# kmjc/PulsePortraiture

Measured on AMD Instinct MI355X. Metric: TOAs/sec (phase+DM fit, 64ch×2048bin fp64) at 1/2/4/8 MI355X, higher is better.
Workload: dtype f64

## Files before the change

include/ppfit.h:

```cpp
#ifndef PPFIT_H
#define PPFIT_H

#include <stdint.h>

#ifdef __cplusplus
extern "C" {
#endif

#define PPF_OK 0
#define PPF_ERR_INVALID -1
#define PPF_ERR_DEVICE -2
#define PPF_ERR_UNSUPPORTED -3
#define PPF_ERR_NOMEM -4

#define PPF_MAX_NCHAN 16384
#define PPF_LDS_NCHAN 2048
#define PPF_VERSION 1

#define PPF_K_MODEL_FFT 0
#define PPF_K_DATA_XSPEC 1
#define PPF_K_SOLVE 2
#define PPF_K_PHASE_SHIFT 3
#define PPF_K_ROTATE 4
#define PPF_K_ROT_ACCUM 5
// ... 17 lines not shown
typedef struct ppf_ctx ppf_ctx;

int ppf_version(void);
int ppf_ctx_create(int device, ppf_ctx** out);
void ppf_ctx_destroy(ppf_ctx* ctx);
const char* ppf_last_error(const ppf_ctx* ctx);
int ppf_set_stream(ppf_ctx* ctx, void* stream);
int ppf_synchronize(ppf_ctx* ctx);
int ppf_set_pipeline(ppf_ctx* ctx, int32_t pieces);
#define PPF_OPT_SCAT_GRAPH 0
#define PPF_OPT_SCAT_SPLIT 1
#define PPF_OPT_SCAT_TAIL 2
#define PPF_OPT_FUSE_MOMENTS 3
#define PPF_OPT_GUESS_WAVE 4
#define PPF_OPT_HBM_TABLES 5
#define PPF_NUM_OPTS 6
int ppf_set_option(ppf_ctx* ctx, int32_t option, int32_t value);
int ppf_get_option(const ppf_ctx* ctx, int32_t option, int32_t* value);
int ppf_set_workspace_limit(ppf_ctx* ctx, int64_t bytes);
int ppf_get_workspace_limit(const ppf_ctx* ctx, int64_t* bytes);
int ppf_set_timing(ppf_ctx* ctx, int enable);
int ppf_set_trace(ppf_ctx* ctx, double* buf, int32_t cap);
int ppf_get_kernel_time(ppf_ctx* ctx, int kernel_id, double* total_ms,
                        int64_t* launches);
int ppf_reset_kernel_times(ppf_ctx* ctx);
int ppf_get_pca_gram_times(ppf_ctx* ctx, double* ms);
#define PPF_SELFTEST_N 10
int ppf_selftest(ppf_ctx* ctx, int32_t* fails);
#define PPF_PHASE_N 32
int ppf_phase_profile(ppf_ctx* ctx, int32_t enable, uint64_t* out);

// ... 247 lines not shown
```

pulseportraiture_amd/_lib.py:

```python
import ctypes
import os

HERE = os.path.dirname(os.path.abspath(__file__))
LIB_PATH = os.path.join(HERE, "libppfit.so")

PPF_OK = 0
PPF_METHOD_TRUST_NCG = 0
PPF_METHOD_TNC = 1
PPF_METHOD_NEWTON_CG = 2
PPF_METHOD_TNC_LEGACY = 3
METHODS = {"trust-ncg": PPF_METHOD_TRUST_NCG, "TNC": PPF_METHOD_TNC,
           "Newton-CG": PPF_METHOD_NEWTON_CG, "TNC-legacy": PPF_METHOD_TNC_LEGACY}
KERNEL_IDS = {"model_fft": 0, "data_xspec": 1, "solve": 2, "phase_shift": 3,
              "rotate": 4, "rot_accum": 5, "synth": 6, "irfft": 7, "noise": 8,
              "guess": 9, "post": 10, "fit_taylor": 11, "moments": 12, "resid": 13, "unpack": 14,
              "pca": 15, "gauss": 16, "pack": 17, "swt": 18, "gbank": 19, "fscrunch": 20}
PPF_THRESH = {"hard": 0, "soft": 1}
PPF_SOLVE_EXACT = 1
PPF_SOLVE_EVAL = 2
PPF_GUESS_DIRECT = 4
PPF_SPEC_NONE = 0
PPF_SPEC_STORE = 1
PPF_SPEC_USE = 2
PPF_SELFTEST_N = 10
GAUSS_STATUS = {1: "converged: ftol", 2: "converged: xtol", 3: "converged: ftol and xtol",
                5: "evaluation cap reached", -1: "singular normal equations",
                -2: "non-finite residual"}
OPTIONS = {"scat_graph": 0, "scat_split": 1, "scat_tail": 2, "fuse_moments": 3, "guess_wave": 4,
           "hbm_tables": 5}
PPF_PHASE_N = 32

_dp = ctypes.c_void_p


class FitDesc(ctypes.Structure):
    _fields_ = [("nsub", ctypes.c_int32), ("nchan", ctypes.c_int32),
                ("nbin", ctypes.c_int32), ("nmodel", ctypes.c_int32),
                ("fit_flags", ctypes.c_int32 * 5),
                ("log10_tau", ctypes.c_int32), ("option", ctypes.c_int32),
                ("method", ctypes.c_int32), ("is_toa", ctypes.c_int32),
                ("guess", ctypes.c_int32), ("guess_Ns", ctypes.c_int32),
                ("guess_wrap", ctypes.c_int32), ("solver_flags", ctypes.c_int32),
                ("data", _dp), ("model", _dp), ("model_idx", _dp),
                ("freqs", _dp), ("errs", _dp), ("chan_mask", _dp),
# ... 149 lines not shown
```

pulseportraiture_amd/build.py:

```python
import hashlib
import os
import subprocess
import sys

HERE = os.path.dirname(os.path.abspath(__file__))
ROOT = os.path.dirname(HERE)
CSRC = os.path.join(HERE, "csrc")
INC = os.path.join(ROOT, "include")
HIPCC = os.environ.get("HIPCC", "/opt/rocm/bin/hipcc")
CXX = os.environ.get("CXX", "g++")

SOURCES = ["ppfit_lib.hip"]
DEPS = ["ppfit_lib.hip", "ppfit_spectra.hip", "ppfit_fit.hip", "ppfit_taylor.hip", "ppfit_tnc.hip",
        "ppfit_ncg.hip", "ppfit_models.hip", "ppfit_generic.hip", "ppfit_noisefit.hip", "ppfit_fscrunch.hip", "ppfit_fake.hip", "ppfit_pca.hip",
        "ppfit_gram.hip",
        "ppfit_gauss.hip", "ppfit_gbank.hip", "ppfit_swt.hip", "ppfit_nbscat.hip", "ppfit_capi.hip",
        "ppfit_kernels.hpp", "ppfit_device.hpp"]
OUT = os.path.join(HERE, "libppfit.so")
FITS_OUT = os.path.join(HERE, "libppfits.so")
TIM_OUT = os.path.join(HERE, "libpptim.so")

HASH_TAG = b"PPF_SRC_HASH="


def _lib_specs():
    hip = ([HIPCC, "--offload-arch=gfx950", "-O3", "-std=c++17", "-fPIC", "-shared", "-I" + INC,
            "-I" + CSRC, os.path.join(CSRC, SOURCES[0])],
           [os.path.join(CSRC, f) for f in DEPS] + [os.path.join(INC, "ppfit.h")])
    fits = ([CXX, "-O2", "-std=c++17", "-fPIC", "-shared", "-Wall", "-I" + INC,
             os.path.join(CSRC, "psrfits.cpp"), os.path.join(CSRC, "psrfits_write.cpp")],
            [os.path.join(CSRC, "psrfits.cpp"), os.path.join(CSRC, "psrfits_write.cpp"),
             os.path.join(INC, "ppfits.h"), os.path.join(INC, "ppfitsw.h")])
# ... 63 lines not shown
```

pulseportraiture_amd/csrc/ppfit_capi.hip:

```cpp
#include <hip/hip_runtime.h>

#include <algorithm>
#include <cmath>
#include <cstdarg>
#include <cstdio>
#include <cstdlib>
#include <cstring>
#include <string>
#include <vector>

#include "ppfit.h"
#include "ppfit_kernels.hpp"

#ifndef PPF_SRC_HASH
#define PPF_SRC_HASH "unbuilt"
#endif
extern "C" __attribute__((visibility("default"), used)) const char ppf_build_tag[] =
    "PPF_SRC_HASH=" PPF_SRC_HASH;

using namespace ppf;

namespace {

struct TimedLaunch {
// ... 30 lines not shown
  int64_t ws_limit = (int64_t)32 << 30;
  TableCache tw, vp;
  Buffer buf[kNumBuffers];
  size_t taylor_static_lds = kUnknown;
  int* active_h = nullptr;
  hipEvent_t scat_ev[2] = {nullptr, nullptr};
  hipStream_t stream2 = nullptr;
  int pipe = 0;
  std::vector<hipEvent_t> sync_events;
  bool phase_prof = false;
  bool timing = false;
  std::vector<TimedLaunch> pending;
  std::vector<hipEvent_t> pool;
  double* trace = nullptr;
  int trace_cap = 0;
  int opt[PPF_NUM_OPTS] = {1, 1, 512, 1, 1, 0};
  double ktime[PPF_NUM_KERNELS] = {0};
  int64_t klaunch[PPF_NUM_KERNELS] = {0};
  double gram_ms[5] = {0.0, 0.0, 0.0, 0.0, 0.0};
};

namespace {

int fail(ppf_ctx* ctx, int code, const char* fmt, ...) {
  char buf[512];
  va_list ap;
  va_start(ap, fmt);
  vsnprintf(buf, sizeof(buf), fmt, ap);
  va_end(ap);
  if (ctx) ctx->err = buf;
  return code;
// ... 341 lines not shown
  return timed_on(ctx, PPF_K_FIT_TAYLOR, st, [&] {
    WIDE_SWITCH(L.wide, {
      if (fa.Dsp) {
        if (mom) hipLaunchKernelGGL((k_fit_taylor<true, true, WD>), g, b, lds, st, fa);
        else hipLaunchKernelGGL((k_fit_taylor<false, true, WD>), g, b, lds, st, fa);
      } else {
        if (mom) hipLaunchKernelGGL((k_fit_taylor<true, false, WD>), g, b, lds, st, fa);
        else hipLaunchKernelGGL((k_fit_taylor<false, false, WD>), g, b, lds, st, fa);
      }
    });
  });
}

int stage_post(ppf_ctx* ctx, hipStream_t st, int n, const FitArgs& fa, const FitLaunch& L) {
  return timed_on(ctx, PPF_K_POST, st, [&] {
    WIDE_SWITCH(L.wide, {
      hipLaunchKernelGGL((k_post<false, WD>), dim3(n), dim3(kBlock), L.lds_meta, st, fa);
      hipLaunchKernelGGL((k_post<true, WD>), dim3(n), dim3(kBlock), L.lds_meta, st, fa);
    });
  });
}

int stage_errs(ppf_ctx* ctx, hipStream_t st, int n, const SpecArgs& sa, double* errs_out) {
  if (!errs_out) return PPF_OK;
  HIPCHK(ctx, hipMemcpyAsync(errs_out + (size_t)sa.sub0 * sa.nchan, sa.sig,
                             (size_t)n * sa.nchan * sizeof(double), hipMemcpyDeviceToDevice, st));
  return PPF_OK;
}

int scat_split_solve(ppf_ctx* ctx, const FitArgs& fa, int nc, int split, size_t lds_scat) {
  const int nchan = fa.nchan;
  double* part = static_cast<double*>(ctx->buf[kSpart].p);
// ... 355 lines not shown
  const bool exact = fit_is_exact(d), taylor = fit_is_taylor(d);
  SpecArgs sa{};
  FitArgs fa{};
  bind_fit_args(ctx, d, o, sa, fa);
  if (int r = fit_tables(ctx, d, sa, fa)) return r;

  const bool wide = nchan > PPF_LDS_NCHAN || ctx->opt[PPF_OPT_HBM_TABLES] != 0;
  FitWorkspace ws(nchan, fa.NHP, taylor, wide, ctx->ws_limit, d->nsub);
  if (int r = ensure(ctx, ctx->buf[kWs], ws.total)) return r;
  ws.base = static_cast<char*>(ctx->buf[kWs].p);
  ws.slice(0, sa, fa);
  const int64_t chunk = ws.chunk;

  L.nbin = nbin;
  L.wide = wide;
  L.lds_meta = wide ? 0 : meta_lds(nchan);
  L.lds_xspec = wide ? 0 : xspec_dyn_lds(nchan);
  fa.tnl = taylor && !wide ? taylor_lds_moments(ctx, nchan, L.lds_meta) : 0;
  fa.tlds = fa.tnl > 0 ? (int)L.lds_meta : 0;
  L.lds_taylor = L.lds_meta + (size_t)nchan * fa.tnl * sizeof(double);
  L.lds_guess =
      (size_t)(fa.NHP + (d->guess ? pfa_scratch_slots(d->guess_Ns, NH) : 0)) * sizeof(double2);
  const bool split_scat = ctx->opt[PPF_OPT_SCAT_SPLIT] && d->fit_flags[3] &&
                          d->method == PPF_METHOD_TRUST_NCG && !wide;
  const int split = std::max(1, std::min(16, nchan / 64));
  L.lds_scat = scat_sweep_lds(nchan, split);
  if (split_scat) {
    if (int r = ensure(ctx, ctx->buf[kSpart],
                       (size_t)chunk * ((nchan + 7) / 8) * kScatPart * sizeof(double) +
                           64 * sizeof(int) + 256))
// ... 1669 lines not shown
```

pulseportraiture_amd/csrc/ppfit_fit.hip:

```cpp
#include "ppfit_kernels.hpp"

namespace ppf {

constexpr int NACC = 10;
static_assert(NACC == kScatAcc, "k_scat_sweep's LDS rows (scat_sweep_lds)");
constexpr double kTwoPi = 2.0 * kPi;
constexpr double kFourPi2 = 4.0 * kPi * kPi;
constexpr double kDconst2 = kDconst * kDconst;

__host__ __device__ constexpr int pair_i(int p) {
  return p < 5 ? 0 : (p < 9 ? 1 : (p < 12 ? 2 : (p < 14 ? 3 : 4)));
}
__host__ __device__ constexpr int pair_j(int p) {
  return p < 5 ? p : (p < 9 ? p - 4 : (p < 12 ? p - 7 : (p < 14 ? p - 9 : 4)));
}

struct Meta {
  int* chan;
  double* fr;
  double* iw2;
  double* pn;
  double* d1;
  double* d2;
  int nok;
};

__device__ __forceinline__ size_t meta_bytes(int nchan) {
  return (size_t)nchan * (5 * sizeof(double) + sizeof(int));
}

__device__ Meta load_meta(const FitArgs& a, int c, int s, unsigned char* dyn, int* s_nok) {
  Meta m;
  const int nchan = a.nchan;
  m.fr = reinterpret_cast<double*>(dyn);
  m.iw2 = m.fr + nchan;
  m.pn = m.iw2 + nchan;
  m.d1 = m.pn + nchan;
  m.d2 = m.d1 + nchan;
  m.chan = reinterpret_cast<int*>(m.d2 + nchan);
  const int tid = threadIdx.x, lane = tid & 63;
  const uint8_t* mask = a.mask ? a.mask + (size_t)s * nchan : nullptr;
  if (tid < 64) {
    int base = 0;
    for (int n0 = 0; n0 < nchan; n0 += 64) {
      const int n = n0 + lane;
// ... 1 lines not shown
      const unsigned long long b = __ballot(ok);
      const int rank = __popcll(b & ((1ull << lane) - 1ull));
      if (ok) m.chan[base + rank] = n;
      base += __popcll(b);
    }
    if (lane == 0) *s_nok = base;
  }
  __syncthreads();
  m.nok = *s_nok;
  const int midx = a.model_idx ? a.model_idx[s] : 0;
  const double half = 0.5 * (double)a.nbin;
  const double P = a.P[s];
  const double* refs = a.st[c].refs;
  const double r0 = 1.0 / (refs[0] * refs[0]);
  const double r1 = 1.0 / (refs[1] * refs[1]);
  for (int j = tid; j < m.nok; j += kBlock) {
    const int n = m.chan[j];
    const double fr = a.freqs[(size_t)s * nchan + n];
    m.fr[j] = fr;
    const double sg = a.sig[(size_t)c * nchan + n];
    m.iw2[j] = 1.0 / (sg * sg * half);
    m.pn[j] = a.pn[(size_t)midx * nchan + n];
    const double f2 = 1.0 / (fr * fr);
    m.d1[j] = kDconst * (f2 - r0) / P;
    m.d2[j] = kDconst2 * (f2 * f2 - r1 * r1) / P;
  }
  __syncthreads();
  return m;
}

__device__ __forceinline__ double pymod1(double x) {
// ... 16 lines not shown
__device__ __forceinline__ void block_sum_vec(double (&v)[N], double (*red)[48]) {
  const int lane = threadIdx.x & 63, w = threadIdx.x >> 6;
#pragma unroll
  for (int i = 0; i < N; ++i) {
    const double t = wave_sum(v[i]);
    if (lane == 0) red[w][i] = t;
  }
  __syncthreads();
#pragma unroll
  for (int i = 0; i < N; ++i) {
    double t = 0.0;
    for (int q = 0; q < kWaves; ++q) t += red[q][i];
    v[i] = t;
  }
  __syncthreads();
}

constexpr int kPipe = 4;

#ifndef PPF_SCAT_U
#define PPF_SCAT_U 4
#endif
#ifndef PPF_SCAT_WG_PER_CU
#define PPF_SCAT_WG_PER_CU 3
#endif

__device__ __forceinline__ void cells_phase(const double2* __restrict__ Xr, int J, int h,
                                            double phif, double* acc) {
  const double2 step = turn_phasor(8.0, phif);
  const double2 zero = cmk(0.0, 0.0);
// ... 345 lines not shown
    ym *= y8;
  }
  double r0, i1, r2;
  switch (h & 3) {
    case 1: r0 = -S0; i1 = S1; r2 = -S2; break;
    case 2: r0 = -S0; i1 = -S1; r2 = -S2; break;
    case 3: r0 = S0; i1 = -S1; r2 = S2; break;
    default: r0 = S0; i1 = S1; r2 = S2; break;
  }
  acc[0] = r0;
  acc[1] = Ks * i1;
  acc[2] = (Ks * Ks) * r2;
  for (int i = 3; i < NACC; ++i) acc[i] = 0.0;
}

__device__ double taylor_reach(const Meta& m, const double* prm, const double* refs,
                               const TaylorSrc& ts, double P, double Ks, double* red) {
  double mx = 0.0;
  for (int j = threadIdx.x; j < m.nok; j += kBlock)
    mx = fmax(mx, fabs(ts.same ? taylor_delta_lin(prm, ts.xc, m.d1[j], m.d2[j])
                               : taylor_delta(prm, refs, ts, m.fr[j], P)));
  mx = wave_max(mx);
  const int lane = threadIdx.x & 63, w = threadIdx.x >> 6;
  if (lane == 0) red[w] = mx;
  __syncthreads();
  double r = red[0];
  for (int i = 1; i < kWaves; ++i) r = fmax(r, red[i]);
  __syncthreads();
  return kTwoPi * Ks * r;
}

__device__ __forceinline__ int flag_mask(const FitArgs& a) {
  int fm = 0;
#pragma unroll
  for (int i = 0; i < 5; ++i) fm |= a.flags[i] ? 1 << i : 0;
  return fm;
}
// ... 61 lines not shown
    bool on = true;
    if (tid == 0) src = 0;
    else if (tid < 4) { src = tid; on = (fm >> (tid - 1)) & 1; }
    else if (tid >= 6) {
      const int p = tid - 6, pi = pair_i(p), pj = pair_j(p);
      if (pj < 3) { src = 4 + (pi == 0 ? pj : 1 + pi + pj); on = (fm >> pi) & (fm >> pj) & 1; }
    }
    double v = 0.0;
    if (src >= 0 && on)
      for (int q = 0; q < kWaves; ++q) v += red[q][src];
    out[tid] = v;
  }
  __syncthreads();
}

template <int MODE, bool SCAT>
__device__ __forceinline__ void sweep(const FitArgs& a, const Meta& m, int c, int s, const double* prm,
                      const double* refs, double P, double* acc_slot, double* out,
                      double (*red)[48], const TaylorSrc& ts, double (*lrow)[48] = nullptr) {
  if constexpr (MODE == 0 && !SCAT) {
    if (ts.T && ts.same) {
      sweep_taylor0(a, m, prm, acc_slot, out, red, ts);
      return;
    }
  }
  const int tid = threadIdx.x, lane = tid & 63, w = tid >> 6;
  const int g8 = lane >> 3, h = lane & 7;
  const int J = a.NHP >> 3;
  const bool log10_tau = a.log10_tau != 0;
  const double tau_lin = SCAT ? (log10_tau ? pow(10.0, prm[3]) : prm[3]) : 0.0;
  const bool scat = SCAT && tau_lin != 0.0;
  const int midx = a.model_idx ? a.model_idx[s] : 0;
  const int fm = flag_mask(a);
  constexpr int NP = MODE == 0 ? 21 : 45;
  double* myrow = nullptr;
  if (lane < NP) red[w][lane] = 0.0;
  if constexpr (MODE == 1) {
    myrow = lrow[w * 8 + g8];
    if (h == 0)
      for (int i = 0; i < NP; ++i) myrow[i] = 0.0;
  }
  __syncthreads();
  const int ngroups = (m.nok + 7) >> 3;
  for (int gi = w; gi < ngroups; gi += kWaves) {
    const int j = gi * 8 + g8;
    const bool valid = j < m.nok;
    const int jj = valid ? j : m.nok - 1;
    const int n = m.chan[jj];
    const double fr = m.fr[jj];
    double acc[NACC];
    if (!SCAT && ts.T) {
      const double dl = ts.same ? taylor_delta_lin(prm, ts.xc, m.d1[jj], m.d2[jj])
                                : taylor_delta(prm, refs, ts, fr, P);
      taylor_cells(ts, n, h, dl, 0.5 * (double)a.nbin, acc);
    } else if (!scat) {
      const double phif = phase_frac(prm, fr, refs, P);
      const double2* Xr = a.X + ((size_t)c * a.nchan + n) * a.NHP;
      cells_phase(Xr, J, h, phif, acc);
    } else {
      const double phif = phase_frac(prm, fr, refs, P);
      const double2* Xr = a.X + ((size_t)c * a.nchan + n) * a.NHP;
      const double* M2r = a.M2 + ((size_t)midx * a.nchan + n) * a.NHP;
      const double taun = tau_lin * pow(fr / refs[2], prm[4]);
      cells_scat<PPF_SCAT_U>(Xr, M2r, J, h, phif, taun, acc);
    }
#pragma unroll
    for (int i = 0; i < NACC; ++i) acc[i] = group8_sum(acc[i]);
    if constexpr (MODE == 0) {
      const double dpre[2] = {m.d1[jj], m.d2[jj]};
      const ChanDeriv d = derive<SCAT>(acc, scat, m.pn[jj], m.iw2[jj], fr, prm, tau_lin, refs,
                                       P, log10_tau, dpre);
      const double q = d.C * d.C / d.S;
      const LanePick L{d.dph[0], d.dph[1], d.dph[2], d.dts[0],
                       d.dts[1], d.d2ts[0], d.d2ts[1], d.d2ts[2]};
      if (h == 0 && valid) {
        double* dst = acc_slot + (size_t)j * NACC;
        for (int i = 0; i < NACC; ++i) dst[i] = acc[i];
      }
#pragma unroll
      for (int r = 0; r < 3; ++r) {
        const double v = chan8_sum(valid ? mode0_term(d, L, q, h + 8 * r, fm) : 0.0);
        const int t = (lane & 7) + 8 * r;
        if (lane >= 8 && lane < 16 && t < NP) red[w][t] += v;
      }
    } else {
      double ct[NP];
#pragma unroll
      for (int i = 0; i < NP; ++i) ct[i] = 0.0;
      if (h == 0 && valid) {
        const ChanDeriv d = derive<SCAT>(acc, scat, m.pn[j], m.iw2[j], fr, prm, tau_lin, refs, P,
                                         log10_tau);
        const double q = d.C * d.C / d.S;
        const double sc = d.C / d.S;
        double cross[5];
#pragma unroll
        for (int i = 0; i < 5; ++i) cross[i] = -2.0 * (dC_(d, i) - sc * dS_(d, i));
        double* dst = a.wsc + ((size_t)c * a.nchan + j) * 8;
        dst[0] = sc;
        dst[1] = d.S;
#pragma unroll
        for (int i = 0; i < 5; ++i) dst[2 + i] = cross[i];
        const double ic = 1.0 / (2.0 * d.S);
#pragma unroll
        for (int p = 0; p < 15; ++p) {
          const int pi = pair_i(p), pj = pair_j(p);
          if (a.flags[pi] && a.flags[pj]) {
            ct[p] = -2.0 * q * ((d2C_(d, pi, pj) / d.C) - (0.5 * d2S_(d, pi, pj) / d.S));
            ct[15 + p] = cross[pi] * cross[pj] * ic;
            ct[30 + p] = Hn_(d, pi, pj);
          }
        }
      }
      if (h == 0 && valid)
#pragma unroll
        for (int i = 0; i < NP; ++i) myrow[i] += ct[i];
    }
  }
  __syncthreads();
  if (tid < NP) {
    double t = 0.0;
    if constexpr (MODE == 0)
      for (int q = 0; q < kWaves; ++q) t += red[q][tid];
    else
      for (int r = 0; r < kWaves * 8; ++r) t += lrow[r][tid];
    out[tid] = t;
  }
  __syncthreads();
}

__device__ __forceinline__ bool fused_taylor(const FitArgs& a, int s) {
  if (!a.T) return false;
  const double t3 = a.init[(size_t)s * 5 + 3];
  const double tl = a.log10_tau ? pow(10.0, t3) : t3;
  return !((tl != 0.0) || a.flags[3]);
}

// ... 1077 lines not shown
    default: break;
  }
}

__device__ __forceinline__ int nz_nsums(int br) {
  switch (br) {
    case NZ_PD: case NZ_PG: case NZ_TA: return 2;
    case NZ_PDT: return 6;
    case NZ_PDG: return 8;
    case NZ_PDGT: return 14;
    case NZ_PDTA: return 22;
    default: return 0;
  }
}

template <int N>
__device__ __forceinline__ void block_sum_first(double (&v)[22], double (*red)[48]) {
  double u[N];
#pragma unroll
  for (int i = 0; i < N; ++i) u[i] = v[i];
  block_sum_vec(u, red);
#pragma unroll
  for (int i = 0; i < N; ++i) v[i] = u[i];
}

__device__ double closest_positive(const double* r, int nr, bool sq, double fmean) {
  double best = NAN, bd = INFINITY;
  for (int i = 0; i < nr; ++i) {
    if (!(r[i] > 0.0)) continue;
    const double x = sq ? sqrt(r[i]) : r[i];
    const double dd = fabs(fmean - x);
    if (dd < bd) { bd = dd; best = x; }
  }
  return best;
}

__device__ int nz_solve(int br, int option, const double* t, double* nz, PostWs& w) {
  switch (br) {
// ... 51 lines not shown
          co[2] = -(A * A * b - a * a * B) - H44 * C * d - H14 * E * f + H44 * b * E +
                  (A * C * f - a * c * F) + H14 * A * d;
          co[3] = 2 * A * a * b + H44 * c * d + H14 * e * f - H44 * b * e - (A * c + a * C) * f -
                  H14 * a * d;
          co[4] = -a * a * b + a * c * f;
          deg = 4;
        }
        return deg;
      }
    } break;
    default: break;
  }
  return 0;
}

struct PostShared {
  PostWs ws;
  double lrow[kWaves * 8][48];
  double prm[5], refs[3], nu[3];
  double out[48];
  double red[kWaves][48];
  double Xinv[25];
  double ifact[kMT];
  int ifit[5];
  int nfit, nok, bad;
  double fmean, Sd;
};

template <bool SCAT, bool W>
__device__ void post_subint(const FitArgs& a, int c, int s, unsigned char* dyn, PostShared& sh) {
  const int tid = threadIdx.x;
  const int nchan = a.nchan;
  const bool prof = a.ptime != nullptr;
  unsigned long long t0 = prof ? wall_clock64() : 0ull;
  auto mark = [&](int i) {
    if (prof) {
      const unsigned long long t1 = wall_clock64();
      if (tid == 0) atomicAdd(&a.ptime[i], t1 - t0);
      t0 = t1;
    }
  };
  const Meta m = load_meta(a, c, s, dyn, &sh.nok);
  const SolveState& st = a.st[c];
  const double P = a.P[s];
  const bool log10_tau = a.log10_tau != 0;
  if (a.mask) {
    for (int n = tid; n < nchan; n += kBlock) {
      if (a.mask[(size_t)s * nchan + n]) continue;
      const size_t o = (size_t)s * nchan + n;
      a.o_scales[o] = 0.0;
      a.o_scale_errs[o] = 0.0;
      a.o_channel_snrs[o] = 0.0;
    }
  }
  {
    double v[2] = {0.0, 0.0};
    for (int j = tid; j < m.nok; j += kBlock) {
      v[0] += a.dsum[(size_t)c * nchan + m.chan[j]] * m.iw2[j];
      v[1] += m.fr[j];
    }
    block_sum_vec(v, sh.red);
    if (tid == 0) { sh.Sd = v[0]; sh.fmean = v[1] / (double)m.nok; }
  }
  if (tid == 0) {
    sh.nfit = 0;
    for (int i = 0; i < 5; ++i) if (a.flags[i]) sh.ifit[sh.nfit++] = i;
    for (int i = 0; i < 3; ++i) sh.refs[i] = st.refs[i];
    sh.bad = (m.nok == 0);
  }
  __syncthreads();
  mark(16);
  if (sh.bad) {
    if (tid == 0) {
      for (int i = 0; i < 5; ++i) {
        a.o_params[(size_t)s * 5 + i] = NAN;
        a.o_param_errs[(size_t)s * 5 + i] = NAN;
      }
// ... 5 lines not shown
  const double* acc_fin = a.acc + ((size_t)c * 2 + st.slot) * nchan * NACC;
  bool need = false;
  double nuo[3];
  for (int i = 0; i < 3; ++i) {
    nuo[i] = a.nu_out[(size_t)s * 3 + i];
    if (isnan(nuo[i]) || nuo[i] == 0.0) need = true;
  }
  if (need) {
    int fl[5];
    for (int i = 0; i < 5; ++i) fl[i] = a.flags[i] ? 1 : 0;
    const int br = nz_branch(fl);
    if (br == NZ_PDTA) fl[2] = 0;
    double t[22];
    double sums[22];
    for (int i = 0; i < 22; ++i) sums[i] = 0.0;
    if (br != NZ_NONE) {
      const double tau_lin = log10_tau ? pow(10.0, st.x[3]) : st.x[3];
      const bool scat = SCAT && tau_lin != 0.0;
      for (int j = tid; j < m.nok; j += kBlock) {
        const ChanDeriv d = derive<SCAT>(acc_fin + (size_t)j * NACC, scat, m.pn[j], m.iw2[j], m.fr[j],
                                   st.x, tau_lin, sh.refs, P, log10_tau);
        nz_terms(br, a.option, d, m.fr[j], sh.refs, fl, t);
        for (int i = 0; i < 22; ++i) sums[i] += t[i];
      }
    }
    switch (nz_nsums(br)) {
      case 2: block_sum_first<2>(sums, sh.red); break;
      case 6: block_sum_first<6>(sums, sh.red); break;
      case 8: block_sum_first<8>(sums, sh.red); break;
      case 14: block_sum_first<14>(sums, sh.red); break;
      case 22: block_sum_first<22>(sums, sh.red); break;
      default: break;
    }
    double* nz = sh.ws.nz;
    if (tid == 0) {
      for (int i = 0; i < 3; ++i) nz[i] = sh.refs[i];
      sh.ws.deg = nz_solve(br, a.option, sums, nz, sh.ws);
    }
    __syncthreads();
    const int pdeg = sh.ws.deg;
    if (pdeg > 0) {
      const int nr = poly_real_roots(sh.ws.co, pdeg, sh.ws, tid);
      if (tid == 0) nz[0] = nz[1] = closest_positive(sh.ws.prev, nr, true, sh.fmean);
    }
    if (tid == 0)
      for (int i = 0; i < 3; ++i) if (isnan(nuo[i])) nuo[i] = nz[i];
  }
// ... 19 lines not shown
    sh.prm[2] = x[2];
    sh.prm[3] = tau_out;
    sh.prm[4] = x[4];
    for (int i = 0; i < 3; ++i) sh.nu[i] = nuo[i];
  }
  __syncthreads();
  TaylorSrc ts{};
  if (!SCAT && st.taylor) {
    const double Ks = 0.5 * (double)a.nbin;
    if (tid < kMT) sh.ifact[tid] = c_inv_fact[tid];
    int best = st.xslot;
    double by = INFINITY;
    for (int q = 0; q < 2; ++q) {
      if (!(st.mvalid & (1 << q))) continue;
      const TaylorSrc tq{a.T + ((size_t)c * 2 + q) * nchan * kMT, st.xc[q], st.refs};
      const double y = taylor_reach(m, sh.prm, sh.nu, tq, P, Ks, sh.red[0]);
      if (y < by) { by = y; best = q; }
    }
    ts = TaylorSrc{a.T + ((size_t)c * 2 + best) * nchan * kMT, st.xc[best], st.refs, false,
                   sh.ifact};
  }
  mark(18);
  sweep<1, SCAT>(a, m, c, s, sh.prm, sh.nu, P, nullptr, sh.out, sh.red, ts, sh.lrow);
  mark(19);
  if (tid == 0) {
    bool fit[5];
#pragma unroll
    for (int i = 0; i < 5; ++i) fit[i] = a.flags[i] != 0;
    double A[5][5], Ai[5][5];
#pragma unroll
    for (int p = 0; p < 15; ++p) {
      const int pi = pair_i(p), pj = pair_j(p);
      A[pi][pj] = A[pj][pi] = sh.out[p] - sh.out[15 + p];
    }
    const bool ok = invert5_fitted(A, fit, Ai);
#pragma unroll
    for (int i = 0; i < 5; ++i)
#pragma unroll
// ... 16 lines not shown
        int r = 0;
#pragma unroll
        for (int j = 0; j < 5; ++j) {
          if (!fit[j]) continue;
          cn[q * 5 + r] = okc ? Ai[i][j] : NAN;
          ++r;
        }
        ++q;
      }
    }
  }
  __syncthreads();
  mark(20);
  const int nf = sh.nfit;
  double snr2 = 0.0;
  for (int j = tid; j < m.nok; j += kBlock) {
    const double* w = a.wsc + ((size_t)c * nchan + j) * 8;
    const double sc = w[0], S = w[1];
    const double ic = 1.0 / (2.0 * S);
    double LL[5], U[5];
#pragma unroll
    for (int q = 0; q < 5; ++q) U[q] = a.flags[q] ? w[2 + q] : 0.0;
#pragma unroll
    for (int q = 0; q < 5; ++q) {
      double t = 0.0;
#pragma unroll
      for (int i = 0; i < 5; ++i)
        if (a.flags[i] && a.flags[q]) t += U[i] * sh.Xinv[i * 5 + q];
      LL[q] = -ic * t;
    }
    double t = 0.0;
#pragma unroll
    for (int q = 0; q < 5; ++q)
      if (a.flags[q]) t += LL[q] * U[q];
    const double LR = -t * ic + ic;
    const double csnr = sc * sqrt(S);
    const int n = m.chan[j];
    const size_t o = (size_t)s * nchan + n;
    a.o_scales[o] = sc;
    a.o_scale_errs[o] = sqrt(2.0 * LR);
    a.o_channel_snrs[o] = csnr;
    snr2 += csnr * csnr;
  }
  snr2 = block_sum(snr2, sh.red[0]);
  if (tid == 0) {
    double* op = a.o_params + (size_t)s * 5;
    double* oe = a.o_param_errs + (size_t)s * 5;
    for (int i = 0; i < 5; ++i) { op[i] = sh.prm[i]; oe[i] = 0.0; }
    double* cv = a.o_cov + (size_t)s * 25;
    for (int i = 0; i < 25; ++i) cv[i] = 0.0;
    int q = 0;
    for (int i = 0; i < 5; ++i) {
      if (!a.flags[i]) continue;
      oe[i] = sqrt(2.0 * sh.Xinv[i * 5 + i]);
      int r = 0;
      for (int j = 0; j < 5; ++j) {
        if (!a.flags[j]) continue;
        cv[q * 5 + r] = 2.0 * sh.Xinv[i * 5 + j];
        ++r;
// ... 9 lines not shown
    a.o_nfev[s] = st.nfev;
    a.o_status[s] = st.status;
    if (a.o_init_used) for (int i = 0; i < 5; ++i) a.o_init_used[(size_t)s * 5 + i] = st.init[i];
    if (a.o_fun) a.o_fun[s] = st.fun;
  }
  mark(21);
  if (prof && tid == 0) atomicAdd(&a.ptime[22], 1ull);
}

template <bool SCAT, bool WIDE>
#ifndef PPF_POST_SCAT_WG_PER_CU
#define PPF_POST_SCAT_WG_PER_CU 2
#endif
__global__ __launch_bounds__(kBlock, SCAT ? PPF_POST_SCAT_WG_PER_CU : PPF_POST_WG_PER_CU) void k_post(FitArgs a) {
  extern __shared__ __align__(16) unsigned char dyn[];
  __shared__ PostShared sh;
  const int c = blockIdx.x, s = a.sub0 + c;
  if ((a.st[c].scat_post != 0) != SCAT) return;
  post_subint<SCAT, WIDE>(a, c, s, chan_tables<WIDE>(a, dyn), sh);
}

}
```

pulseportraiture_amd/csrc/ppfit_kernels.hpp:

```cpp
#pragma once
#include "ppfit.h"
#include "ppfit_device.hpp"

namespace ppf {

struct SpecArgs {
  int sub0, nchan, NHP, kc, guess;
  int log10_tau, fit_tau, exact;
  int spec_mode;
  const double* data;
  const double2* M;
  const int* model_idx;
  const double* freqs;
  const double* errs;
  const uint8_t* mask;
  const double* weights;
  const double* P;
  const double* init;
  const double* guess_nu;
  double2* X;
  double2* R;
  double* sig;
  double* dsum;
  const double2* tw;
// ... 57 lines not shown
  int taylor;
  double xc[2][5];
  int mvalid, xslot;
  double g[5], H[25], tr;
  double xp[5], pl[5], predv;
  int hits, kit, sdone;
};

struct FitArgs {
  int sub0, nchan, nbin, NH, NHP, kc;
  int flags[5];
  int log10_tau, option, is_toa, guess, Ns, guess_wrap;
  int solver_flags;
  int method;
  int guess_wave;
  const double2* X;
  const double2* Dsp;
  const double2* R;
  const double2* M;
  const double* M2;
  const double* pn;
  const int* model_idx;
  const double* sig;
  const double* dsum;
  const double* freqs;
  const uint8_t* mask;
  const double* P;
  const double* init;
  const double* nu_fit;
  const double* nu_out;
// ... 20 lines not shown
  double* o_channel_snrs;
  double* o_chi2;
  double* o_red_chi2;
  double* o_snr;
  int* o_nfev;
  int* o_status;
  double* o_init_used;
  double* o_fun;
  double* o_cov_nosc;
  double* o_grad;
  double* o_hess;
  double bounds[5][2];
  unsigned char* gdyn;
  size_t gdyn_stride;
};

constexpr int kTraceRec = 32;
__device__ __forceinline__ void trace_sweep(const FitArgs& a, int s, int isweep, const double* x,
                                            const double* out, int nout, bool counted) {
  if (!a.trace || threadIdx.x != 0 || isweep >= a.trace_cap) return;
  double* r = a.trace + ((size_t)s * a.trace_cap + isweep) * kTraceRec;
  for (int i = 0; i < 5; ++i) r[i] = x[i];
  for (int i = 0; i < 21; ++i) r[5 + i] = i < nout ? out[i] : NAN;
  r[26] = counted ? 1.0 : 0.0;
  r[27] = (double)isweep;
}

struct GuessShared {
  double red[kWaves];
  double bestv[kWaves];
// ... 635 lines not shown
  return scat_meta_lds(nchan) + rows * (kScatAcc * sizeof(double) + 2 * sizeof(double));
}
__global__ void k_scat_sweep(FitArgs a, double* part, int split, int init);
__global__ void k_scat_step(FitArgs a, const double* part, int init, int* ctrs, int par);
__global__ void k_model_mean(const double2* M, double2* Mmean, int nchan, int NHP);
template <bool MOM, bool DSP, bool WIDE = false>
__global__ void k_fit_taylor(FitArgs a);
template <int U, bool DSP>
__global__ void k_moments(FitArgs a);
__global__ void k_selftest(int* fails);
template <bool SCAT, bool WIDE = false> __global__ void k_solve(FitArgs a);
template <bool SCAT, bool WIDE = false> __global__ void k_tnc(FitArgs a);
template <bool SCAT, bool WIDE = false> __global__ void k_ncg(FitArgs a);
__global__ void k_guess_w(FitArgs a);
template <bool SCAT, bool WIDE = false> __global__ void k_post(FitArgs a);

}
```

Measured before the change: 1.266 million.

## Run non-scattering post stage on single-wave workgroups via virtual-thread emulation

Adds a 64-thread k_post_w kernel that handles the non-scattering post-fit stage for small channel counts when Taylor tables are present and tau is not fitted. Each wave loops over virtual wave slots, so the block-wide reductions and syncs become wave-level sums. The point is to stop wasting a full block with heavy LDS on only 64 channels and to raise occupancy. The cost is serialised slot loops within one wave, plus a duplicate code path controlled by a new option that is on by default.

Measured after the change: 1.305 million, median of 6. 3.1% higher.

```diff
diff --git a/include/ppfit.h b/include/ppfit.h
--- a/include/ppfit.h
+++ b/include/ppfit.h
@@ -55,7 +55,8 @@
 #define PPF_OPT_FUSE_MOMENTS 3
 #define PPF_OPT_GUESS_WAVE 4
 #define PPF_OPT_HBM_TABLES 5
-#define PPF_NUM_OPTS 6
+#define PPF_OPT_POST_WAVE 6
+#define PPF_NUM_OPTS 7
 int ppf_set_option(ppf_ctx* ctx, int32_t option, int32_t value);
 int ppf_get_option(const ppf_ctx* ctx, int32_t option, int32_t* value);
 int ppf_set_workspace_limit(ppf_ctx* ctx, int64_t bytes);
diff --git a/pulseportraiture_amd/_lib.py b/pulseportraiture_amd/_lib.py
--- a/pulseportraiture_amd/_lib.py
+++ b/pulseportraiture_amd/_lib.py
@@ -27,7 +27,7 @@
                 5: "evaluation cap reached", -1: "singular normal equations",
                 -2: "non-finite residual"}
 OPTIONS = {"scat_graph": 0, "scat_split": 1, "scat_tail": 2, "fuse_moments": 3, "guess_wave": 4,
-           "hbm_tables": 5}
+           "hbm_tables": 5, "post_wave": 6}
 PPF_PHASE_N = 32
 
 _dp = ctypes.c_void_p
diff --git a/pulseportraiture_amd/build.py b/pulseportraiture_amd/build.py
--- a/pulseportraiture_amd/build.py
+++ b/pulseportraiture_amd/build.py
@@ -15,7 +15,7 @@
         "ppfit_ncg.hip", "ppfit_models.hip", "ppfit_generic.hip", "ppfit_noisefit.hip", "ppfit_fscrunch.hip", "ppfit_fake.hip", "ppfit_pca.hip",
         "ppfit_gram.hip",
         "ppfit_gauss.hip", "ppfit_gbank.hip", "ppfit_swt.hip", "ppfit_nbscat.hip", "ppfit_capi.hip",
-        "ppfit_kernels.hpp", "ppfit_device.hpp"]
+        "ppfit_kernels.hpp", "ppfit_device.hpp", "ppfit_vthread.hpp"]
 OUT = os.path.join(HERE, "libppfit.so")
 FITS_OUT = os.path.join(HERE, "libppfits.so")
 TIM_OUT = os.path.join(HERE, "libpptim.so")
diff --git a/pulseportraiture_amd/csrc/ppfit_capi.hip b/pulseportraiture_amd/csrc/ppfit_capi.hip
--- a/pulseportraiture_amd/csrc/ppfit_capi.hip
+++ b/pulseportraiture_amd/csrc/ppfit_capi.hip
@@ -68,7 +68,7 @@
   std::vector<hipEvent_t> pool;
   double* trace = nullptr;
   int trace_cap = 0;
-  int opt[PPF_NUM_OPTS] = {1, 1, 512, 1, 1, 0};
+  int opt[PPF_NUM_OPTS] = {1, 1, 512, 1, 1, 0, 1};
   double ktime[PPF_NUM_KERNELS] = {0};
   int64_t klaunch[PPF_NUM_KERNELS] = {0};
   double gram_ms[5] = {0.0, 0.0, 0.0, 0.0, 0.0};
@@ -440,8 +440,10 @@
 
 int stage_post(ppf_ctx* ctx, hipStream_t st, int n, const FitArgs& fa, const FitLaunch& L) {
   return timed_on(ctx, PPF_K_POST, st, [&] {
+    if (post_wave_ok(fa)) hipLaunchKernelGGL(k_post_w, dim3(n), dim3(64), L.lds_meta, st, fa);
     WIDE_SWITCH(L.wide, {
-      hipLaunchKernelGGL((k_post<false, WD>), dim3(n), dim3(kBlock), L.lds_meta, st, fa);
+      if (!post_wave_ok(fa))
+        hipLaunchKernelGGL((k_post<false, WD>), dim3(n), dim3(kBlock), L.lds_meta, st, fa);
       hipLaunchKernelGGL((k_post<true, WD>), dim3(n), dim3(kBlock), L.lds_meta, st, fa);
     });
   });
@@ -827,6 +829,7 @@
 
   L.nbin = nbin;
   L.wide = wide;
+  fa.post_wave = ctx->opt[PPF_OPT_POST_WAVE] && !wide;
   L.lds_meta = wide ? 0 : meta_lds(nchan);
   L.lds_xspec = wide ? 0 : xspec_dyn_lds(nchan);
   fa.tnl = taylor && !wide ? taylor_lds_moments(ctx, nchan, L.lds_meta) : 0;
diff --git a/pulseportraiture_amd/csrc/ppfit_fit.hip b/pulseportraiture_amd/csrc/ppfit_fit.hip
--- a/pulseportraiture_amd/csrc/ppfit_fit.hip
+++ b/pulseportraiture_amd/csrc/ppfit_fit.hip
@@ -1,4 +1,5 @@
 #include "ppfit_kernels.hpp"
+#include "ppfit_vthread.hpp"
 
 namespace ppf {
 
@@ -29,6 +30,7 @@
   return (size_t)nchan * (5 * sizeof(double) + sizeof(int));
 }
 
+template <int NT = kBlock>
 __device__ Meta load_meta(const FitArgs& a, int c, int s, unsigned char* dyn, int* s_nok) {
   Meta m;
   const int nchan = a.nchan;
@@ -60,7 +62,7 @@
   const double* refs = a.st[c].refs;
   const double r0 = 1.0 / (refs[0] * refs[0]);
   const double r1 = 1.0 / (refs[1] * refs[1]);
-  for (int j = tid; j < m.nok; j += kBlock) {
+  for (int j = tid; j < m.nok; j += NT) {
     const int n = m.chan[j];
     const double fr = a.freqs[(size_t)s * nchan + n];
     m.fr[j] = fr;
@@ -107,6 +109,24 @@
     v[i] = t;
   }
   __syncthreads();
+}
+
+template <int NT, int N>
+__device__ __forceinline__ void vt_sum_vec(double (&v)[N], double (&tot)[N], double (*red)[48]) {
+  if constexpr (NT == kBlock) {
+    block_sum_vec(v, red);
+#pragma unroll
+    for (int i = 0; i < N; ++i) tot[i] = v[i];
+  } else {
+#pragma unroll
+    for (int i = 0; i < N; ++i) tot[i] += wave_sum(v[i]);
+  }
+}
+
+template <int NT>
+__device__ __forceinline__ double vt_sum(double v, double tot, double* red) {
+  if constexpr (NT == kBlock) return block_sum(v, red);
+  else return tot + wave_sum(v);
 }
 
 constexpr int kPipe = 4;
@@ -482,13 +502,15 @@
   for (int i = 3; i < NACC; ++i) acc[i] = 0.0;
 }
 
+template <int NT = kBlock>
 __device__ double taylor_reach(const Meta& m, const double* prm, const double* refs,
                                const TaylorSrc& ts, double P, double Ks, double* red) {
   double mx = 0.0;
-  for (int j = threadIdx.x; j < m.nok; j += kBlock)
+  for (int j = threadIdx.x; j < m.nok; j += NT)
     mx = fmax(mx, fabs(ts.same ? taylor_delta_lin(prm, ts.xc, m.d1[j], m.d2[j])
                                : taylor_delta(prm, refs, ts, m.fr[j], P)));
   mx = wave_max(mx);
+  if constexpr (NT == 64) return kTwoPi * Ks * mx;
   const int lane = threadIdx.x & 63, w = threadIdx.x >> 6;
   if (lane == 0) red[w] = mx;
   __syncthreads();
@@ -580,17 +602,19 @@
   __syncthreads();
 }
 
-template <int MODE, bool SCAT>
+template <int MODE, bool SCAT, int NT = kBlock>
 __device__ __forceinline__ void sweep(const FitArgs& a, const Meta& m, int c, int s, const double* prm,
                       const double* refs, double P, double* acc_slot, double* out,
                       double (*red)[48], const TaylorSrc& ts, double (*lrow)[48] = nullptr) {
+  static_assert(NT == kBlock || (MODE == 1 && kBlock % NT == 0 && NT % 64 == 0),
+                "only the with-scales sweep runs on virtual waves");
   if constexpr (MODE == 0 && !SCAT) {
     if (ts.T && ts.same) {
       sweep_taylor0(a, m, prm, acc_slot, out, red, ts);
       return;
     }
   }
-  const int tid = threadIdx.x, lane = tid & 63, w = tid >> 6;
+  const int tid = threadIdx.x, lane = tid & 63, rw = tid >> 6;
   const int g8 = lane >> 3, h = lane & 7;
   const int J = a.NHP >> 3;
   const bool log10_tau = a.log10_tau != 0;
@@ -600,92 +624,105 @@
   const int fm = flag_mask(a);
   constexpr int NP = MODE == 0 ? 21 : 45;
   double* myrow = nullptr;
-  if (lane < NP) red[w][lane] = 0.0;
-  if constexpr (MODE == 1) {
-    myrow = lrow[w * 8 + g8];
-    if (h == 0)
-      for (int i = 0; i < NP; ++i) myrow[i] = 0.0;
-  }
-  __syncthreads();
   const int ngroups = (m.nok + 7) >> 3;
-  for (int gi = w; gi < ngroups; gi += kWaves) {
-    const int j = gi * 8 + g8;
-    const bool valid = j < m.nok;
-    const int jj = valid ? j : m.nok - 1;
-    const int n = m.chan[jj];
-    const double fr = m.fr[jj];
-    double acc[NACC];
-    if (!SCAT && ts.T) {
-      const double dl = ts.same ? taylor_delta_lin(prm, ts.xc, m.d1[jj], m.d2[jj])
-                                : taylor_delta(prm, refs, ts, fr, P);
-      taylor_cells(ts, n, h, dl, 0.5 * (double)a.nbin, acc);
-    } else if (!scat) {
-      const double phif = phase_frac(prm, fr, refs, P);
-      const double2* Xr = a.X + ((size_t)c * a.nchan + n) * a.NHP;
-      cells_phase(Xr, J, h, phif, acc);
-    } else {
-      const double phif = phase_frac(prm, fr, refs, P);
-      const double2* Xr = a.X + ((size_t)c * a.nchan + n) * a.NHP;
-      const double* M2r = a.M2 + ((size_t)midx * a.nchan + n) * a.NHP;
-      const double taun = tau_lin * pow(fr / refs[2], prm[4]);
-      cells_scat<PPF_SCAT_U>(Xr, M2r, J, h, phif, taun, acc);
-    }
-#pragma unroll
-    for (int i = 0; i < NACC; ++i) acc[i] = group8_sum(acc[i]);
-    if constexpr (MODE == 0) {
-      const double dpre[2] = {m.d1[jj], m.d2[jj]};
-      const ChanDeriv d = derive<SCAT>(acc, scat, m.pn[jj], m.iw2[jj], fr, prm, tau_lin, refs,
-                                       P, log10_tau, dpre);
-      const double q = d.C * d.C / d.S;
-      const LanePick L{d.dph[0], d.dph[1], d.dph[2], d.dts[0],
-                       d.dts[1], d.d2ts[0], d.d2ts[1], d.d2ts[2]};
-      if (h == 0 && valid) {
-        double* dst = acc_slot + (size_t)j * NACC;
-        for (int i = 0; i < NACC; ++i) dst[i] = acc[i];
-      }
-#pragma unroll
-      for (int r = 0; r < 3; ++r) {
-        const double v = chan8_sum(valid ? mode0_term(d, L, q, h + 8 * r, fm) : 0.0);
-        const int t = (lane & 7) + 8 * r;
-        if (lane >= 8 && lane < 16 && t < NP) red[w][t] += v;
-      }
-    } else {
-      double ct[NP];
-#pragma unroll
-      for (int i = 0; i < NP; ++i) ct[i] = 0.0;
-      if (h == 0 && valid) {
-        const ChanDeriv d = derive<SCAT>(acc, scat, m.pn[j], m.iw2[j], fr, prm, tau_lin, refs, P,
-                                         log10_tau);
+  const int nslot = NT == kBlock ? 1 : vt_live_slots(ngroups, kWaves, NT / 64);
+  double tot = 0.0;
+  for (int sl = 0; sl < nslot; ++sl) {
+    const int w = vt_wave(rw, sl, NT);
+    if constexpr (NT == kBlock)
+      if (lane < NP) red[w][lane] = 0.0;
+    if constexpr (MODE == 1) {
+      myrow = lrow[NT == kBlock ? ws_row(w, g8) : ws_local_row(rw, g8)];
+      if (h == 0)
+        for (int i = 0; i < NP; ++i) myrow[i] = 0.0;
+    }
+    __syncthreads();
+    for (int gi = ws_first_group(w); gi < ngroups; gi += kWaves) {
+      const int j = gi * 8 + g8;
+      const bool valid = j < m.nok;
+      const int jj = valid ? j : m.nok - 1;
+      const int n = m.chan[jj];
+      const double fr = m.fr[jj];
+      double acc[NACC];
+      if (!SCAT && ts.T) {
+        const double dl = ts.same ? taylor_delta_lin(prm, ts.xc, m.d1[jj], m.d2[jj])
+                                  : taylor_delta(prm, refs, ts, fr, P);
+        taylor_cells(ts, n, h, dl, 0.5 * (double)a.nbin, acc);
+      } else if (!scat) {
+        const double phif = phase_frac(prm, fr, refs, P);
+        const double2* Xr = a.X + ((size_t)c * a.nchan + n) * a.NHP;
+        cells_phase(Xr, J, h, phif, acc);
+      } else {
+        const double phif = phase_frac(prm, fr, refs, P);
+        const double2* Xr = a.X + ((size_t)c * a.nchan + n) * a.NHP;
+        const double* M2r = a.M2 + ((size_t)midx * a.nchan + n) * a.NHP;
+        const double taun = tau_lin * pow(fr / refs[2], prm[4]);
+        cells_scat<PPF_SCAT_U>(Xr, M2r, J, h, phif, taun, acc);
+      }
+#pragma unroll
+      for (int i = 0; i < NACC; ++i) acc[i] = group8_sum(acc[i]);
+      if constexpr (MODE == 0) {
+        const double dpre[2] = {m.d1[jj], m.d2[jj]};
+        const ChanDeriv d = derive<SCAT>(acc, scat, m.pn[jj], m.iw2[jj], fr, prm, tau_lin, refs,
+                                         P, log10_tau, dpre);
         const double q = d.C * d.C / d.S;
-        const double sc = d.C / d.S;
-        double cross[5];
-#pragma unroll
-        for (int i = 0; i < 5; ++i) cross[i] = -2.0 * (dC_(d, i) - sc * dS_(d, i));
-        double* dst = a.wsc + ((size_t)c * a.nchan + j) * 8;
-        dst[0] = sc;
-        dst[1] = d.S;
-#pragma unroll
-        for (int i = 0; i < 5; ++i) dst[2 + i] = cross[i];
-        const double ic = 1.0 / (2.0 * d.S);
-#pragma unroll
-        for (int p = 0; p < 15; ++p) {
-          const int pi = pair_i(p), pj = pair_j(p);
-          if (a.flags[pi] && a.flags[pj]) {
-            ct[p] = -2.0 * q * ((d2C_(d, pi, pj) / d.C) - (0.5 * d2S_(d, pi, pj) / d.S));
-            ct[15 + p] = cross[pi] * cross[pj] * ic;
-            ct[30 + p] = Hn_(d, pi, pj);
+        const LanePick L{d.dph[0], d.dph[1], d.dph[2], d.dts[0],
+                         d.dts[1], d.d2ts[0], d.d2ts[1], d.d2ts[2]};
+        if (h == 0 && valid) {
+          double* dst = acc_slot + (size_t)j * NACC;
+          for (int i = 0; i < NACC; ++i) dst[i] = acc[i];
+        }
+#pragma unroll
+        for (int r = 0; r < 3; ++r) {
+          const double v = chan8_sum(valid ? mode0_term(d, L, q, h + 8 * r, fm) : 0.0);
+          const int t = (lane & 7) + 8 * r;
+          if (lane >= 8 && lane < 16 && t < NP) red[w][t] += v;
+        }
+      } else {
+        double ct[NP];
+#pragma unroll
+        for (int i = 0; i < NP; ++i) ct[i] = 0.0;
+        if (h == 0 && valid) {
+          const ChanDeriv d = derive<SCAT>(acc, scat, m.pn[j], m.iw2[j], fr, prm, tau_lin, refs, P,
+                                           log10_tau);
+          const double q = d.C * d.C / d.S;
+          const double sc = d.C / d.S;
+          double cross[5];
+#pragma unroll
+          for (int i = 0; i < 5; ++i) cross[i] = -2.0 * (dC_(d, i) - sc * dS_(d, i));
+          double* dst = a.wsc + ((size_t)c * a.nchan + j) * 8;
+          dst[0] = sc;
+          dst[1] = d.S;
+#pragma unroll
+          for (int i = 0; i < 5; ++i) dst[2 + i] = cross[i];
+          const double ic = 1.0 / (2.0 * d.S);
+#pragma unroll
+          for (int p = 0; p < 15; ++p) {
+            const int pi = pair_i(p), pj = pair_j(p);
+            if (a.flags[pi] && a.flags[pj]) {
+              ct[p] = -2.0 * q * ((d2C_(d, pi, pj) / d.C) - (0.5 * d2S_(d, pi, pj) / d.S));
+              ct[15 + p] = cross[pi] * cross[pj] * ic;
+              ct[30 + p] = Hn_(d, pi, pj);
+            }
           }
         }
-      }
-      if (h == 0 && valid)
-#pragma unroll
-        for (int i = 0; i < NP; ++i) myrow[i] += ct[i];
-    }
-  }
-  __syncthreads();
+        if (h == 0 && valid)
+#pragma unroll
+          for (int i = 0; i < NP; ++i) myrow[i] += ct[i];
+      }
+    }
+    __syncthreads();
+    if constexpr (NT < kBlock) {
+      if (tid < NP)
+        for (int r = 0; r < (NT / 64) * 8; ++r) tot += lrow[r][tid];
+      __syncthreads();
+    }
+  }
   if (tid < NP) {
     double t = 0.0;
-    if constexpr (MODE == 0)
+    if constexpr (NT < kBlock)
+      t = tot;
+    else if constexpr (MODE == 0)
       for (int q = 0; q < kWaves; ++q) t += red[q][tid];
     else
       for (int r = 0; r < kWaves * 8; ++r) t += lrow[r][tid];
@@ -1793,14 +1830,15 @@
   }
 }
 
-template <int N>
-__device__ __forceinline__ void block_sum_first(double (&v)[22], double (*red)[48]) {
-  double u[N];
-#pragma unroll
-  for (int i = 0; i < N; ++i) u[i] = v[i];
-  block_sum_vec(u, red);
-#pragma unroll
-  for (int i = 0; i < N; ++i) v[i] = u[i];
+template <int N, int NT = kBlock>
+__device__ __forceinline__ void block_sum_first(double (&v)[22], double (&tot)[22],
+                                                double (*red)[48]) {
+  double u[N], t[N];
+#pragma unroll
+  for (int i = 0; i < N; ++i) { u[i] = v[i]; t[i] = tot[i]; }
+  vt_sum_vec<NT>(u, t, red);
+#pragma unroll
+  for (int i = 0; i < N; ++i) tot[i] = t[i];
 }
 
 __device__ double closest_positive(const double* r, int nr, bool sq, double fmean) {
@@ -1882,12 +1920,13 @@
   return 0;
 }
 
+template <int NT = kBlock>
 struct PostShared {
   PostWs ws;
-  double lrow[kWaves * 8][48];
+  double lrow[(NT / 64) * 8][48];
   double prm[5], refs[3], nu[3];
   double out[48];
-  double red[kWaves][48];
+  double red[NT / 64][48];
   double Xinv[25];
   double ifact[kMT];
   int ifit[5];
@@ -1895,8 +1934,8 @@
   double fmean, Sd;
 };
 
-template <bool SCAT, bool W>
-__device__ void post_subint(const FitArgs& a, int c, int s, unsigned char* dyn, PostShared& sh) {
+template <bool SCAT, bool W, int NT = kBlock>
+__device__ void post_subint(const FitArgs& a, int c, int s, unsigned char* dyn, PostShared<NT>& sh) {
   const int tid = threadIdx.x;
   const int nchan = a.nchan;
   const bool prof = a.ptime != nullptr;
@@ -1908,12 +1947,13 @@
       t0 = t1;
     }
   };
-  const Meta m = load_meta(a, c, s, dyn, &sh.nok);
+  const Meta m = load_meta<NT>(a, c, s, dyn, &sh.nok);
   const SolveState& st = a.st[c];
   const double P = a.P[s];
   const bool log10_tau = a.log10_tau != 0;
+  const int nslot = NT == kBlock ? 1 : vt_live_slots(m.nok, kBlock, NT);
   if (a.mask) {
-    for (int n = tid; n < nchan; n += kBlock) {
+    for (int n = tid; n < nchan; n += NT) {
       if (a.mask[(size_t)s * nchan + n]) continue;
       const size_t o = (size_t)s * nchan + n;
       a.o_scales[o] = 0.0;
@@ -1922,13 +1962,16 @@
     }
   }
   {
-    double v[2] = {0.0, 0.0};
-    for (int j = tid; j < m.nok; j += kBlock) {
-      v[0] += a.dsum[(size_t)c * nchan + m.chan[j]] * m.iw2[j];
-      v[1] += m.fr[j];
-    }
-    block_sum_vec(v, sh.red);
-    if (tid == 0) { sh.Sd = v[0]; sh.fmean = v[1] / (double)m.nok; }
+    double tot[2] = {0.0, 0.0};
+    for (int q = 0; q < nslot; ++q) {
+      double v[2] = {0.0, 0.0};
+      for (int j = vt_thread(tid, q, NT); j < m.nok; j += kBlock) {
+        v[0] += a.dsum[(size_t)c * nchan + m.chan[j]] * m.iw2[j];
+        v[1] += m.fr[j];
+      }
+      vt_sum_vec<NT>(v, tot, sh.red);
+    }
+    if (tid == 0) { sh.Sd = tot[0]; sh.fmean = tot[1] / (double)m.nok; }
   }
   if (tid == 0) {
     sh.nfit = 0;
@@ -1964,23 +2007,27 @@
     double t[22];
     double sums[22];
     for (int i = 0; i < 22; ++i) sums[i] = 0.0;
-    if (br != NZ_NONE) {
-      const double tau_lin = log10_tau ? pow(10.0, st.x[3]) : st.x[3];
-      const bool scat = SCAT && tau_lin != 0.0;
-      for (int j = tid; j < m.nok; j += kBlock) {
-        const ChanDeriv d = derive<SCAT>(acc_fin + (size_t)j * NACC, scat, m.pn[j], m.iw2[j], m.fr[j],
-                                   st.x, tau_lin, sh.refs, P, log10_tau);
-        nz_terms(br, a.option, d, m.fr[j], sh.refs, fl, t);
-        for (int i = 0; i < 22; ++i) sums[i] += t[i];
-      }
-    }
-    switch (nz_nsums(br)) {
-      case 2: block_sum_first<2>(sums, sh.red); break;
-      case 6: block_sum_first<6>(sums, sh.red); break;
-      case 8: block_sum_first<8>(sums, sh.red); break;
-      case 14: block_sum_first<14>(sums, sh.red); break;
-      case 22: block_sum_first<22>(sums, sh.red); break;
-      default: break;
+    for (int q = 0; q < nslot; ++q) {
+      double part[22];
+      for (int i = 0; i < 22; ++i) part[i] = 0.0;
+      if (br != NZ_NONE) {
+        const double tau_lin = log10_tau ? pow(10.0, st.x[3]) : st.x[3];
+        const bool scat = SCAT && tau_lin != 0.0;
+        for (int j = vt_thread(tid, q, NT); j < m.nok; j += kBlock) {
+          const ChanDeriv d = derive<SCAT>(acc_fin + (size_t)j * NACC, scat, m.pn[j], m.iw2[j], m.fr[j],
+                                     st.x, tau_lin, sh.refs, P, log10_tau);
+          nz_terms(br, a.option, d, m.fr[j], sh.refs, fl, t);
+          for (int i = 0; i < 22; ++i) part[i] += t[i];
+        }
+      }
+      switch (nz_nsums(br)) {
+        case 2: block_sum_first<2, NT>(part, sums, sh.red); break;
+        case 6: if constexpr (NT == kBlock) block_sum_first<6, NT>(part, sums, sh.red); break;
+        case 8: block_sum_first<8, NT>(part, sums, sh.red); break;
+        case 14: if constexpr (NT == kBlock) block_sum_first<14, NT>(part, sums, sh.red); break;
+        case 22: if constexpr (NT == kBlock) block_sum_first<22, NT>(part, sums, sh.red); break;
+        default: break;
+      }
     }
     double* nz = sh.ws.nz;
     if (tid == 0) {
@@ -2030,14 +2077,14 @@
     for (int q = 0; q < 2; ++q) {
       if (!(st.mvalid & (1 << q))) continue;
       const TaylorSrc tq{a.T + ((size_t)c * 2 + q) * nchan * kMT, st.xc[q], st.refs};
-      const double y = taylor_reach(m, sh.prm, sh.nu, tq, P, Ks, sh.red[0]);
+      const double y = taylor_reach<NT>(m, sh.prm, sh.nu, tq, P, Ks, sh.red[0]);
       if (y < by) { by = y; best = q; }
     }
     ts = TaylorSrc{a.T + ((size_t)c * 2 + best) * nchan * kMT, st.xc[best], st.refs, false,
                    sh.ifact};
   }
   mark(18);
-  sweep<1, SCAT>(a, m, c, s, sh.prm, sh.nu, P, nullptr, sh.out, sh.red, ts, sh.lrow);
+  sweep<1, SCAT, NT>(a, m, c, s, sh.prm, sh.nu, P, nullptr, sh.out, sh.red, ts, sh.lrow);
   mark(19);
   if (tid == 0) {
     bool fit[5];
@@ -2084,35 +2131,38 @@
   mark(20);
   const int nf = sh.nfit;
   double snr2 = 0.0;
-  for (int j = tid; j < m.nok; j += kBlock) {
-    const double* w = a.wsc + ((size_t)c * nchan + j) * 8;
-    const double sc = w[0], S = w[1];
-    const double ic = 1.0 / (2.0 * S);
-    double LL[5], U[5];
-#pragma unroll
-    for (int q = 0; q < 5; ++q) U[q] = a.flags[q] ? w[2 + q] : 0.0;
-#pragma unroll
-    for (int q = 0; q < 5; ++q) {
+  for (int vq = 0; vq < nslot; ++vq) {
+    double part = 0.0;
+    for (int j = vt_thread(tid, vq, NT); j < m.nok; j += kBlock) {
+      const double* w = a.wsc + ((size_t)c * nchan + j) * 8;
+      const double sc = w[0], S = w[1];
+      const double ic = 1.0 / (2.0 * S);
+      double LL[5], U[5];
+#pragma unroll
+      for (int q = 0; q < 5; ++q) U[q] = a.flags[q] ? w[2 + q] : 0.0;
+#pragma unroll
+      for (int q = 0; q < 5; ++q) {
+        double t = 0.0;
+#pragma unroll
+        for (int i = 0; i < 5; ++i)
+          if (a.flags[i] && a.flags[q]) t += U[i] * sh.Xinv[i * 5 + q];
+        LL[q] = -ic * t;
+      }
       double t = 0.0;
 #pragma unroll
-      for (int i = 0; i < 5; ++i)
-        if (a.flags[i] && a.flags[q]) t += U[i] * sh.Xinv[i * 5 + q];
-      LL[q] = -ic * t;
-    }
-    double t = 0.0;
-#pragma unroll
-    for (int q = 0; q < 5; ++q)
-      if (a.flags[q]) t += LL[q] * U[q];
-    const double LR = -t * ic + ic;
-    const double csnr = sc * sqrt(S);
-    const int n = m.chan[j];
-    const size_t o = (size_t)s * nchan + n;
-    a.o_scales[o] = sc;
-    a.o_scale_errs[o] = sqrt(2.0 * LR);
-    a.o_channel_snrs[o] = csnr;
-    snr2 += csnr * csnr;
-  }
-  snr2 = block_sum(snr2, sh.red[0]);
+      for (int q = 0; q < 5; ++q)
+        if (a.flags[q]) t += LL[q] * U[q];
+      const double LR = -t * ic + ic;
+      const double csnr = sc * sqrt(S);
+      const int n = m.chan[j];
+      const size_t o = (size_t)s * nchan + n;
+      a.o_scales[o] = sc;
+      a.o_scale_errs[o] = sqrt(2.0 * LR);
+      a.o_channel_snrs[o] = csnr;
+      part += csnr * csnr;
+    }
+    snr2 = vt_sum<NT>(part, snr2, sh.red[0]);
+  }
   if (tid == 0) {
     double* op = a.o_params + (size_t)s * 5;
     double* oe = a.o_param_errs + (size_t)s * 5;
@@ -2152,10 +2202,23 @@
 #endif
 __global__ __launch_bounds__(kBlock, SCAT ? PPF_POST_SCAT_WG_PER_CU : PPF_POST_WG_PER_CU) void k_post(FitArgs a) {
   extern __shared__ __align__(16) unsigned char dyn[];
-  __shared__ PostShared sh;
+  __shared__ PostShared<> sh;
   const int c = blockIdx.x, s = a.sub0 + c;
   if ((a.st[c].scat_post != 0) != SCAT) return;
+  if constexpr (!SCAT)
+    if (post_wave_ok(a)) return;
   post_subint<SCAT, WIDE>(a, c, s, chan_tables<WIDE>(a, dyn), sh);
 }
 
-}
+#ifndef PPF_POST_WAVE_OCC
+#define PPF_POST_WAVE_OCC 12
+#endif
+__global__ __launch_bounds__(64, PPF_POST_WAVE_OCC) void k_post_w(FitArgs a) {
+  extern __shared__ __align__(16) unsigned char dyn[];
+  __shared__ PostShared<64> sh;
+  const int c = blockIdx.x, s = a.sub0 + c;
+  if (!post_wave_ok(a) || a.st[c].scat_post != 0) return;
+  post_subint<false, false, 64>(a, c, s, dyn, sh);
+}
+
+}
diff --git a/pulseportraiture_amd/csrc/ppfit_kernels.hpp b/pulseportraiture_amd/csrc/ppfit_kernels.hpp
--- a/pulseportraiture_amd/csrc/ppfit_kernels.hpp
+++ b/pulseportraiture_amd/csrc/ppfit_kernels.hpp
@@ -95,6 +95,7 @@
   int solver_flags;
   int method;
   int guess_wave;
+  int post_wave;
   const double2* X;
   const double2* Dsp;
   const double2* R;
@@ -145,6 +146,14 @@
   unsigned char* gdyn;
   size_t gdyn_stride;
 };
+
+#ifndef PPF_POST_WAVE_NCHAN
+#define PPF_POST_WAVE_NCHAN 128
+#endif
+constexpr int kPostWaveNchan = PPF_POST_WAVE_NCHAN;
+__host__ __device__ inline bool post_wave_ok(const FitArgs& a) {
+  return a.post_wave && a.T && a.nchan <= kPostWaveNchan && !a.flags[3] && !a.flags[4];
+}
 
 constexpr int kTraceRec = 32;
 __device__ __forceinline__ void trace_sweep(const FitArgs& a, int s, int isweep, const double* x,
@@ -810,5 +819,6 @@
 template <bool SCAT, bool WIDE = false> __global__ void k_ncg(FitArgs a);
 __global__ void k_guess_w(FitArgs a);
 template <bool SCAT, bool WIDE = false> __global__ void k_post(FitArgs a);
-
-}
+__global__ void k_post_w(FitArgs a);
+
+}
diff --git a/pulseportraiture_amd/csrc/ppfit_vthread.hpp b/pulseportraiture_amd/csrc/ppfit_vthread.hpp
--- /dev/null
+++ b/pulseportraiture_amd/csrc/ppfit_vthread.hpp
@@ -0,0 +1,24 @@
+#pragma once
+
+#if defined(__HIPCC__)
+#define PPF_HD __host__ __device__
+#else
+#define PPF_HD
+#endif
+
+namespace ppf {
+
+PPF_HD constexpr int vt_slots(int block, int nt) { return block / nt; }
+PPF_HD constexpr int vt_thread(int tid, int q, int nt) { return tid + nt * q; }
+PPF_HD constexpr int vt_wave(int w, int q, int nt) { return w + (nt / 64) * q; }
+PPF_HD constexpr int vt_live_slots(int n, int block, int nt) {
+  const int all = vt_slots(block, nt), need = (n + nt - 1) / nt;
+  return need < 1 ? 1 : (need < all ? need : all);
+}
+
+PPF_HD constexpr int ws_row(int vw, int g8) { return vw * 8 + g8; }
+PPF_HD constexpr int ws_first_group(int vw) { return vw; }
+PPF_HD constexpr int ws_chan(int gi, int g8) { return gi * 8 + g8; }
+PPF_HD constexpr int ws_local_row(int w, int g8) { return w * 8 + g8; }
+
+}
```
